# microsoft/fadtk

Hardware: NVIDIA H100
Metric: audio_seconds_embedded_per_second (higher is better)
Workload: dtype f16

## Files before the change

fadtk_b200/csrc/conv_gemm.cuh:

```cuda
#pragma once
#include "sm90.cuh"

namespace fad {

struct ConvGemmParams {
    int taps;
    int cblks;
    int box_w, box_h, box_n;
    int tiles_w, tiles_h;
    int img_groups;
    int n_tiles;
    int H, W, NB, Cout;
    float lo_scale;
    int lo8_group;
    int ld_out, n_valid;
    int relu, pool;
    const float* bias;
    __half* out;
    float* out_f32;
    uint8_t* out8;
    float* resid;
    int resid_C, resid_res, resid_shift;
};

// ... 1 lines not shown
    const int lg_nw = 28 - __clz(res);
    const int nw = res >> 3;
    const int in = (int)(o & 63);
    const long long wi = o >> 6;
    const int wx = (int)wi & (nw - 1);
    const int wy = (int)(wi >> lg_nw) & (nw - 1);
    const long long b = wi >> (2 * lg_nw);
    int y = wy * 8 + (in >> 3) + shift, xx = wx * 8 + (in & 7) + shift;
    if (y >= res) y -= res;
    if (xx >= res) xx -= res;
    return (b * res + y) * res + xx;
}

constexpr int kTileM = 128;
constexpr int kBlockK = 64;
constexpr int kConvGemmThreads = 384;
constexpr int kConsumers = 2;
constexpr int kChunkSteps = 8;
constexpr float kAccumShrinkPerElement = 1.06e-9f;
constexpr uint32_t kABytes = kTileM * kBlockK * 2;
constexpr uint32_t kEpiRowBytes = 128 * 4;
constexpr uint32_t kEpiBytes = 64 * kEpiRowBytes;
constexpr uint32_t kStagingBytes = 32 * 128;

template <int N_TILE, int WMODE>
__host__ __device__ constexpr uint32_t conv_gemm_stage_bytes() {
    return WMODE == 2 ? kABytes + N_TILE * kBlockK * 2 + N_TILE * kBlockK + kTileM * kBlockK
                      : kABytes + (WMODE == 1 ? 2 : 1) * N_TILE * kBlockK * 2;
}

template <int N_TILE, int STAGES, int WMODE>
__host__ __device__ constexpr uint32_t conv_gemm_smem_bytes() {
    return STAGES * conv_gemm_stage_bytes<N_TILE, WMODE>() + 1024  + 256
         + kConsumers * kEpiBytes;
}

__device__ __forceinline__ uint32_t pack_half2(float a, float b) {
    __half2 h = __floats2half2_rn(a, b);
    return *reinterpret_cast<uint32_t*>(&h);
}
__device__ __forceinline__ float gelu_erf(float x) {
    const float z = fminf(fabsf(x) * 0.70710678118654752f, 4.3f);
    float q = 1.04899843e-04f;
    q = fmaf(q, z, -4.92790774e-04f);
    q = fmaf(q, z, -2.22368206e-03f);
    q = fmaf(q, z, 2.93586859e-02f);
    q = fmaf(q, z, -1.48908889e-01f);
    q = fmaf(q, z, -9.18342944e-01f);
    q = fmaf(q, z, -1.62791250e+00f);
// ... 13 lines not shown
    __half2_raw h0, h1;
    h0.x = (unsigned short)(a & 0xffffu); h0.y = (unsigned short)(a >> 16);
    h1.x = (unsigned short)(b & 0xffffu); h1.y = (unsigned short)(b >> 16);
    return (uint32_t)__nv_cvt_halfraw2_to_fp8x2(h0, __NV_SATFINITE, __NV_E4M3)
         | ((uint32_t)__nv_cvt_halfraw2_to_fp8x2(h1, __NV_SATFINITE, __NV_E4M3) << 16);
}
__device__ __forceinline__ uint2 f16x8_to_e4m3x8(uint4 v) {
    return make_uint2(f16x4_to_e4m3x4(v.x, v.y), f16x4_to_e4m3x4(v.z, v.w));
}

__device__ __forceinline__ uint32_t hmax2_u32(uint32_t a, uint32_t b) {
    __half2 r = __hmax2(*reinterpret_cast<__half2*>(&a), *reinterpret_cast<__half2*>(&b));
    return *reinterpret_cast<uint32_t*>(&r);
}

template <int N_TILE, int STAGES, int WMODE>
__global__ void __launch_bounds__(kConvGemmThreads, 1)
conv_gemm_kernel(const __grid_constant__ CUtensorMap map_x,
                 const __grid_constant__ CUtensorMap map_w,
                 const __grid_constant__ CUtensorMap map_wl8,
                 const __grid_constant__ CUtensorMap map_x8,
                 const ConvGemmParams p)
{
    using namespace sm90;
    static_assert(N_TILE == 128, "one m64n128 accumulator per consumer warpgroup");
    constexpr bool SPLIT_W = WMODE == 1;
    constexpr bool LO8 = WMODE == 2;
    constexpr uint32_t kStageBytes = conv_gemm_stage_bytes<N_TILE, WMODE>();
    constexpr int kBRows = (WMODE != 0 ? 2 : 1) * N_TILE;
    constexpr uint32_t kWhBytes = N_TILE * kBlockK * 2;
    constexpr uint32_t kOffWl8 = kABytes + kWhBytes;
    constexpr uint32_t kOffA8 = kOffWl8 + N_TILE * kBlockK;
    constexpr int kColsPerThread = N_TILE / 2;
    constexpr int kGroups = kColsPerThread / 32;

    extern __shared__ uint8_t smem_raw[];
    uint8_t* smem = reinterpret_cast<uint8_t*>((reinterpret_cast<uintptr_t>(smem_raw) + 1023) & ~uintptr_t(1023));
    uint64_t* bars = reinterpret_cast<uint64_t*>(smem + STAGES * kStageBytes);
    uint64_t* full = bars;
    uint64_t* empty = bars + STAGES;
    uint8_t* epi = smem + STAGES * kStageBytes + 256;

    const int warp = threadIdx.x >> 5;
    const int lane = threadIdx.x & 31;
    const int ksteps = p.taps * p.cblks;
    const int n_chunks = (ksteps + kChunkSteps - 1) / kChunkSteps;
    const int chunk_len = (ksteps + n_chunks - 1) / n_chunks;
    const int m_tiles = p.img_groups * p.tiles_h * p.tiles_w;
    const int total_tiles = m_tiles * p.n_tiles;

    if (warp == 0 && lane == 0) {
        tma_prefetch_desc(&map_x);
        tma_prefetch_desc(&map_w);
        if (LO8) { tma_prefetch_desc(&map_wl8); tma_prefetch_desc(&map_x8); }
    }
    if (warp == 1 && lane == 0) {
        for (int s = 0; s < STAGES; ++s) { mbar_init(&full[s], 1); mbar_init(&empty[s], kConsumers * 4); }
        mbar_fence_init();
    }
    __syncthreads();

    if (warp < 4) {
        setmaxnreg_dec<40>();
        if (warp == 0 && elect_one()) {
            int s = 0; uint32_t ph = 0;
            for (int tile = blockIdx.x; tile < total_tiles; tile += gridDim.x) {
                const int nt = tile % p.n_tiles;
                const int m = tile / p.n_tiles;
                const int w0 = (m % p.tiles_w) * p.box_w;
                const int h0 = ((m / p.tiles_w) % p.tiles_h) * p.box_h;
                const int n0 = (m / (p.tiles_w * p.tiles_h)) * p.box_n;
                for (int ks = 0; ks < ksteps; ++ks) {
                    const int tap = ks / p.cblks;
                    const int cb = ks - tap * p.cblks;
                    int dh = 0, dw = 0;
                    if (p.taps == 9) { dh = tap / 3 - 1; dw = tap % 3 - 1; }
                    mbar_wait(&empty[s], ph ^ 1);
                    uint8_t* st = smem + s * kStageBytes;
                    mbar_expect_tx(&full[s], kStageBytes);
                    tma_load_4d(st, &map_x, &full[s], cb * kBlockK, w0 + dw, h0 + dh, n0);
                    tma_load_2d(st + kABytes, &map_w, &full[s], ks * kBlockK, nt * kBRows);
                    if (LO8) {
                        tma_load_2d(st + kOffWl8, &map_wl8, &full[s], ks * kBlockK, nt * N_TILE);
                        tma_load_4d(st + kOffA8, &map_x8, &full[s], cb * kBlockK, w0 + dw, h0 + dh, n0);
                    }
                    if (++s == STAGES) { s = 0; ph ^= 1; }
                }
            }
        }
    } else {
        setmaxnreg_inc<232>();
        const int c = (warp >> 2) - 1;
        const int wg_t = threadIdx.x & 127;
        const int wq = wg_t >> 5;
        const int rr = wg_t & 63;
        const int half = wg_t >> 6;
        const int r = c * 64 + rr;
        const int bw = p.box_w, bh = p.box_h;
        const int pw = r % bw;
        const int phh = (r / bw) % bh;
        const int pn = r / (bw * bh);
        const uint32_t epi_base = smem_u32(epi) + c * kEpiBytes;
        const uint32_t bar_id = 1 + c;
        int s = 0; uint32_t ph = 0;
        const bool plain = p.tiles_w == 1 && p.tiles_h == 1 && bw == 1 && bh == 1;
        auto prefetch_resid = [&](int nt_, int m_) {
            if (p.resid == nullptr || !plain) return;
            const int n_ = m_ * kTileM + r;
            if (n_ >= p.NB) return;
            const long long tok = p.resid_res ? window_row_to_token((long long)n_, p.resid_res, p.resid_shift) : (long long)n_;
            const int c0 = nt_ * N_TILE + half * kColsPerThread;
            for (int cc = c0; cc < c0 + kColsPerThread && cc < p.resid_C; cc += 32)
                asm volatile("prefetch.global.L2 [%0];" :: "l"(p.resid + tok * p.resid_C + cc));
        };
        if ((int)blockIdx.x < total_tiles) prefetch_resid((int)blockIdx.x % p.n_tiles, (int)blockIdx.x / p.n_tiles);
        auto load_bias = [&](float4 (&b)[8], int col0) {
            const float4* src = reinterpret_cast<const float4*>(p.bias + col0);
#pragma unroll
            for (int j = 0; j < 8; ++j) b[j] = __ldg(src + j);
        };

        for (int tile = blockIdx.x; tile < total_tiles; tile += gridDim.x) {
            const int nt = tile % p.n_tiles;
            const int m = tile / p.n_tiles;
            if (tile + (int)gridDim.x < total_tiles)
                prefetch_resid((tile + (int)gridDim.x) % p.n_tiles, (tile + (int)gridDim.x) / p.n_tiles);

            float sum[64], acc[64], corr[LO8 ? 64 : 1];
#pragma unroll
            for (int i = 0; i < 64; ++i) sum[i] = 0.f;
            for (int ks0 = 0; ks0 < ksteps; ks0 += chunk_len) {
                const int ks1 = min(ks0 + chunk_len, ksteps);
                const float unshrink = kAccumShrinkPerElement * (float)((ks1 - ks0) * kBlockK);
                int prev_s = -1;
                for (int ks = ks0; ks < ks1; ++ks) {
                    mbar_wait(&full[s], ph);
                    const uint32_t a_addr = smem_u32(smem + s * kStageBytes);
                    const uint64_t a_desc = kmajor_sw128_desc(a_addr + c * 64 * 128);
                    const uint64_t b_desc = kmajor_sw128_desc(a_addr + kABytes);
                    wgmma_fence();
#pragma unroll
                    for (int k = 0; k < kBlockK / 16; ++k) {
                        wgmma_m64n128k16_f16<0, 0>(acc, a_desc + 2 * k, b_desc + 2 * k, (ks > ks0) || (k > 0));
                        if (SPLIT_W)
                            wgmma_m64n128k16_f16<0, 0>(acc, a_desc + 2 * k, b_desc + 2 * k + (N_TILE * 128 / 16), 1);
                    }
                    if constexpr (LO8) {
                        const uint64_t a8_desc = kmajor_sw64_desc(a_addr + kOffA8 + c * 64 * 64);
                        const uint64_t w8_desc = kmajor_sw64_desc(a_addr + kOffWl8);
#pragma unroll
                        for (int k = 0; k < kBlockK / 32; ++k)
                            wgmma_m64n128k32_e4m3(corr, a8_desc + 2 * k, w8_desc + 2 * k, (ks > 0) || (k > 0));
                    }
                    wgmma_commit();
                    wgmma_wait<1>();
                    if (prev_s >= 0) { __syncwarp(); if (lane == 0) mbar_arrive(&empty[prev_s]); }
                    prev_s = s;
                    if (++s == STAGES) { s = 0; ph ^= 1; }
                }
                wgmma_wait<0>();
                fence_regs(acc);
                if constexpr (LO8) fence_regs(corr);
                __syncwarp();
                if (lane == 0) mbar_arrive(&empty[prev_s]);
#pragma unroll
                for (int i = 0; i < 64; ++i) sum[i] += fmaf(acc[i], unshrink, acc[i]);
            }
            if constexpr (LO8) {
#pragma unroll
                for (int i = 0; i < 64; ++i) sum[i] = fmaf(corr[i], p.lo_scale, sum[i]);
            }

            named_bar_sync(bar_id, 128);
            {
                const int fr = wq * 16 + (lane >> 2);
#pragma unroll
                for (int j = 0; j < 16; ++j) {
#pragma unroll
                    for (int i = 0; i < 2; ++i) {
                        const int row = fr + 8 * i, col = 8 * j + 2 * (lane & 3);
                        const uint32_t addr = epi_base + row * kEpiRowBytes + ((((col >> 2) ^ (row & 7))) << 4) + (col & 3) * 4;
                        sts64(addr, sum[4 * j + 2 * i], sum[4 * j + 2 * i + 1]);
                    }
                }
            }
            named_bar_sync(bar_id, 128);
            float accr[kColsPerThread];
#pragma unroll
            for (int q4 = 0; q4 < kColsPerThread / 4; ++q4) {
                const int ch = half * (kColsPerThread / 4) + q4;
                const uint4 u = lds128(epi_base + rr * kEpiRowBytes + ((ch ^ (rr & 7)) << 4));
                accr[4 * q4 + 0] = __uint_as_float(u.x); accr[4 * q4 + 1] = __uint_as_float(u.y);
                accr[4 * q4 + 2] = __uint_as_float(u.z); accr[4 * q4 + 3] = __uint_as_float(u.w);
            }
            named_bar_sync(bar_id, 128);

            int w, h, n;
            if (plain) { w = 0; h = 0; n = m * kTileM + r; }
            else {
                w = (m % p.tiles_w) * bw + pw;
                h = ((m / p.tiles_w) % p.tiles_h) * bh + phh;
                n = (m / (p.tiles_w * p.tiles_h)) * p.box_n + pn;
            }
            const bool valid = n < p.NB;
            const int ch0 = nt * N_TILE + half * kColsPerThread;
            long long out_off = -1, res_off = -1;
            if (valid && !p.pool) {
                out_off = (long long)((size_t(n) * p.H + h) * p.W + w) * p.ld_out;
                if (p.resid != nullptr)
                    res_off = (p.resid_res ? window_row_to_token((long long)n, p.resid_res, p.resid_shift) : (long long)n)
                              * p.resid_C;
            }
            const uint32_t stg = epi_base + wq * kStagingBytes;
            const uint32_t stg_mine = stg + lane * 128;
            const int sw = lane & 7;
            const int cq = lane & 7, rq = lane >> 3;
            const bool f32_path = p.out_f32 != nullptr || p.resid != nullptr;
            float4 bnext[8];
#pragma unroll
            for (int g = 0; g < kGroups; ++g) {
                float f[32];
                load_bias(bnext, ch0 + g * 32);
#pragma unroll
                for (int j = 0; j < 8; ++j) {
                    const float4 b = bnext[j];
                    f[4 * j + 0] = accr[g * 32 + 4 * j + 0] + b.x;
                    f[4 * j + 1] = accr[g * 32 + 4 * j + 1] + b.y;
                    f[4 * j + 2] = accr[g * 32 + 4 * j + 2] + b.z;
                    f[4 * j + 3] = accr[g * 32 + 4 * j + 3] + b.w;
                }
                if (p.relu == 1) {
#pragma unroll
                    for (int j = 0; j < 32; ++j) f[j] = fmaxf(f[j], 0.0f);
                } else if (p.relu == 2) {
#pragma unroll
                    for (int j = 0; j < 32; ++j) f[j] = gelu_erf(f[j]);
                } else if (p.relu == 3) {
#pragma unroll
                    for (int j = 0; j < 32; ++j) f[j] = elu_ex2(f[j]);
                }
                uint32_t h2[16];
#pragma unroll
                for (int j = 0; j < 16; ++j) h2[j] = pack_half2(f[2 * j], f[2 * j + 1]);

                if (!p.pool) {
                    if (f32_path) {
#pragma unroll
                        for (int j = 0; j < 8; ++j)
                            sts128(stg_mine + ((j ^ sw) << 4), __float_as_uint(f[4 * j]), __float_as_uint(f[4 * j + 1]),
                                   __float_as_uint(f[4 * j + 2]), __float_as_uint(f[4 * j + 3]));
                        __syncwarp();
                        float4 v[8];
#pragma unroll
                        for (int it = 0; it < 8; ++it) {
                            const int rr = it * 4 + rq;
                            const uint4 u = lds128(stg + rr * 128 + ((cq ^ (rr & 7)) << 4));
                            v[it] = make_float4(__uint_as_float(u.x), __uint_as_float(u.y), __uint_as_float(u.z), __uint_as_float(u.w));
                        }
                        const int col = ch0 + g * 32 + cq * 4;
                        if (p.out_f32 != nullptr) {
#pragma unroll
                            for (int it = 0; it < 8; ++it) {
                                const long long off = __shfl_sync(0xffffffffu, out_off, it * 4 + rq);
                                if (off >= 0 && col < p.n_valid) *reinterpret_cast<float4*>(p.out_f32 + off + col) = v[it];
                            }
                        }
                        if (p.resid != nullptr && ch0 + g * 32 < p.resid_C) {
#pragma unroll
                            for (int hf = 0; hf < 2; ++hf) {
                                long long offs[4];
                                float4 xv[4];
#pragma unroll
                                for (int it = 0; it < 4; ++it) {
                                    offs[it] = __shfl_sync(0xffffffffu, res_off, (hf * 4 + it) * 4 + rq);
                                    if (offs[it] >= 0) xv[it] = *reinterpret_cast<const float4*>(p.resid + offs[it] + col);
                                }
#pragma unroll
                                for (int it = 0; it < 4; ++it) {
                                    if (offs[it] >= 0) {
                                        const float4 a = v[hf * 4 + it];
                                        xv[it].x += a.x; xv[it].y += a.y; xv[it].z += a.z; xv[it].w += a.w;
                                        *reinterpret_cast<float4*>(p.resid + offs[it] + col) = xv[it];
                                    }
                                }
                            }
                        }
                        __syncwarp();
                        if (p.out != nullptr && out_off >= 0 && ch0 + g * 32 + 32 <= p.n_valid) {
                            uint4* dst = reinterpret_cast<uint4*>(p.out + out_off + ch0 + g * 32);
#pragma unroll
                            for (int j = 0; j < 4; ++j)
                                dst[j] = make_uint4(h2[4 * j], h2[4 * j + 1], h2[4 * j + 2], h2[4 * j + 3]);
                        }
                    } else if (p.out != nullptr) {
#pragma unroll
                        for (int j = 0; j < 4; ++j)
                            sts128(stg_mine + ((((g & 1) * 4 + j) ^ sw) << 4), h2[4 * j], h2[4 * j + 1], h2[4 * j + 2], h2[4 * j + 3]);
                        if (g & 1) {
                            __syncwarp();
                            const int col = ch0 + (g - 1) * 32 + cq * 8;
#pragma unroll
                            for (int it = 0; it < 8; ++it) {
                                const int rr = it * 4 + rq;
                                const uint4 v = lds128(stg + rr * 128 + ((cq ^ (rr & 7)) << 4));
                                const long long off = __shfl_sync(0xffffffffu, out_off, rr);
                                if (off >= 0 && col < p.n_valid) {
                                    *reinterpret_cast<uint4*>(p.out + off + col) = v;
                                    if (p.out8 != nullptr) *reinterpret_cast<uint2*>(p.out8 + off + col) = f16x8_to_e4m3x8(v);
                                }
                            }
                            __syncwarp();
                        }
                    }
                } else {
#pragma unroll
                    for (int j = 0; j < 16; ++j) {
                        uint32_t o = __shfl_xor_sync(0xffffffffu, h2[j], 1);
                        h2[j] = hmax2_u32(h2[j], o);
                        o = __shfl_xor_sync(0xffffffffu, h2[j], bw);
                        h2[j] = hmax2_u32(h2[j], o);
                    }
                    const int sub = (pw & 1) | ((phh & 1) << 1);
                    uint4 o;
                    o.x = sub == 0 ? h2[0] : sub == 1 ? h2[4] : sub == 2 ? h2[8]  : h2[12];
                    o.y = sub == 0 ? h2[1] : sub == 1 ? h2[5] : sub == 2 ? h2[9]  : h2[13];
                    o.z = sub == 0 ? h2[2] : sub == 1 ? h2[6] : sub == 2 ? h2[10] : h2[14];
                    o.w = sub == 0 ? h2[3] : sub == 1 ? h2[7] : sub == 2 ? h2[11] : h2[15];
                    if (valid) {
                        const size_t pix = (size_t(n) * (p.H >> 1) + (h >> 1)) * (p.W >> 1) + (w >> 1);
                        *reinterpret_cast<uint4*>(p.out + pix * p.Cout + ch0 + g * 32 + sub * 8) = o;
                        if (p.out8 != nullptr) *reinterpret_cast<uint2*>(p.out8 + pix * p.Cout + ch0 + g * 32 + sub * 8) = f16x8_to_e4m3x8(o);
                    }
                }
            }
        }
    }
}

}
```

fadtk_b200/csrc/fadtk_b200.cu:

```cuda
#include "../../include/fadtk_b200.h"

#include <cuda.h>
#include <cuda_runtime.h>
#include <cuda_fp16.h>
#include <cuda_fp8.h>
#include <algorithm>
#include <cmath>
#include <cstdio>
#include <cstdlib>
#include <cstring>
#include <map>
#include <string>
#include <vector>

#include "conv_gemm.cuh"
#include "frontend.cuh"
#include "stats.cuh"
#include "frechet.cuh"
#include "frechet_batched.cuh"
#include "clap.cuh"
#include "resample.cuh"
#include "whisper.cuh"
#include "encodec.cuh"
#include "wav2vec.cuh"
// ... 138 lines not shown
};

namespace {

template <int N_TILE, int STAGES, int WMODE>
int launch_conv_gemm(fad_handle* h, const CUtensorMap& mx, const CUtensorMap& mw, const CUtensorMap& mw8,
                     const CUtensorMap& mx8, const fad::ConvGemmParams& p, cudaStream_t st) {
    static bool attr_set = false;
    constexpr uint32_t smem = fad::conv_gemm_smem_bytes<N_TILE, STAGES, WMODE>();
    static_assert(smem <= 227 * 1024, "over the per-CTA shared-memory limit");
    auto kern = fad::conv_gemm_kernel<N_TILE, STAGES, WMODE>;
    if (!attr_set) {
        CK(cudaFuncSetAttribute(kern, cudaFuncAttributeMaxDynamicSharedMemorySize, (int)smem));
        attr_set = true;
    }
    const int total = p.img_groups * p.tiles_h * p.tiles_w * p.n_tiles;
    if (total == 0) return 0;
    const int grid = total < h->num_sms ? total : h->num_sms;
    kern<<<grid, fad::kConvGemmThreads, smem, st>>>(mx, mw, mw8, mx8, p);
    CK(cudaGetLastError());
    h->launches++;
    return 0;
}

int encode_layer_maps(const LayerGeom& g, const void* x, long long nb_dim, const void* w,
                      CUtensorMap* mx, CUtensorMap* mw, int a_cols = 0, long long a_row_stride = 0) {
    const uint64_t ac = a_cols > 0 ? (uint64_t)a_cols : (uint64_t)g.Cin;
    const uint64_t xd[4] = {ac, (uint64_t)g.W, (uint64_t)g.H, (uint64_t)nb_dim};
    uint64_t xs[3] = {ac * 2, (uint64_t)g.W * ac * 2, (uint64_t)g.H * g.W * ac * 2};
    if (a_row_stride > 0) xs[0] = xs[1] = xs[2] = (uint64_t)a_row_stride * 2;
    const uint32_t xb[4] = {64, (uint32_t)g.box_w, (uint32_t)g.box_h, (uint32_t)g.box_n};
    if (encode_f16_map(mx, x, 4, xd, xs, xb)) return 1;
    const uint64_t K = (uint64_t)g.taps * g.Cin;
    const uint64_t rows_mul = g.split_w ? 2 : 1;
    const uint64_t wd[2] = {K, (uint64_t)g.Cout * rows_mul};
    const uint64_t ws[1] = {K * 2};
    const uint32_t wb[2] = {64, (uint32_t)(g.n_tile * (g.split_w == 1 ? 2 : 1))};
    return encode_f16_map(mw, w, 2, wd, ws, wb);
}

int lo8_for(fad_handle* h, const LayerGeom& g, const void* w, CUtensorMap* mw8, float* inv_scale, cudaStream_t st);

bool attention_wgmma_enabled() {
    static const bool on = [] { const char* e = getenv("FADTK_ATTN"); return !(e && std::string(e) == "legacy"); }();
    return on;
}
int launch_attention_wgmma(fad_handle* h, const __half* qkv, long long n_clips, int S, int d, int heads, __half* out, cudaStream_t st) {
    static bool attr_set = false;
    if (!attr_set) {
        CK(cudaFuncSetAttribute(fad::attention_wgmma_kernel, cudaFuncAttributeMaxDynamicSharedMemorySize, (int)fad::kAtSmem));
        attr_set = true;
    }
// ... 977 lines not shown
```

fadtk_b200/csrc/sm90.cuh:

```cuda
#pragma once
#include <cuda.h>
#include <cuda_fp16.h>
#include <stdint.h>
#include <stdio.h>

namespace sm90 {

__device__ __forceinline__ uint32_t smem_u32(const void* p) {
    return static_cast<uint32_t>(__cvta_generic_to_shared(p));
}
__device__ __forceinline__ uint32_t lane_id() { return threadIdx.x & 31; }

__device__ __forceinline__ bool elect_one() {
    uint32_t pred;
    asm volatile(
        "{\n\t.reg .pred P;\n\t"
        "elect.sync _|P, 0xffffffff;\n\t"
        "selp.u32 %0, 1, 0, P;\n\t}\n"
        : "=r"(pred));
    return pred != 0;
}

template <uint32_t kRegs> __device__ __forceinline__ void setmaxnreg_inc() {
    asm volatile("setmaxnreg.inc.sync.aligned.u32 %0;" ::"n"(kRegs));
// ... 45 lines not shown
    asm volatile(
        "{\n\t.reg .pred P;\n\t"
        "mbarrier.try_wait.parity.shared::cta.b64 P, [%1], %2, %3;\n\t"
        "selp.u32 %0, 1, 0, P;\n\t}\n"
        : "=r"(ok) : "r"(smem_u32(bar)), "r"(parity), "r"(ns) : "memory");
    return ok != 0;
}
__device__ __forceinline__ void mbar_wait(uint64_t* bar, uint32_t parity) {
    if (mbar_try_wait(bar, parity)) return;
    uint32_t spins = 0;
    while (!mbar_try_wait_hint(bar, parity, 2000u)) {
        if (++spins > (1u << 24)) asm volatile("trap;");
    }
}

__device__ __forceinline__ void fence_proxy_async_smem() {
    asm volatile("fence.proxy.async.shared::cta;" ::: "memory");
}

__device__ __forceinline__ void tma_prefetch_desc(const CUtensorMap* m) {
    asm volatile("prefetch.tensormap [%0];" ::"l"(reinterpret_cast<uint64_t>(m)) : "memory");
}
__device__ __forceinline__ void tma_load_2d(void* dst, const CUtensorMap* m, uint64_t* bar,
                                            int c0, int c1) {
    asm volatile(
        "cp.async.bulk.tensor.2d.shared::cluster.global.mbarrier::complete_tx::bytes"
        " [%0], [%1, {%3, %4}], [%2];"
        ::"r"(smem_u32(dst)), "l"(reinterpret_cast<uint64_t>(m)), "r"(smem_u32(bar)),
          "r"(c0), "r"(c1) : "memory");
}
__device__ __forceinline__ void tma_load_3d(void* dst, const CUtensorMap* m, uint64_t* bar,
                                            int c0, int c1, int c2) {
    asm volatile(
        "cp.async.bulk.tensor.3d.shared::cluster.global.mbarrier::complete_tx::bytes"
        " [%0], [%1, {%3, %4, %5}], [%2];"
        ::"r"(smem_u32(dst)), "l"(reinterpret_cast<uint64_t>(m)), "r"(smem_u32(bar)),
          "r"(c0), "r"(c1), "r"(c2) : "memory");
}
__device__ __forceinline__ void tma_load_4d(void* dst, const CUtensorMap* m, uint64_t* bar,
                                            int c0, int c1, int c2, int c3) {
    asm volatile(
        "cp.async.bulk.tensor.4d.shared::cluster.global.mbarrier::complete_tx::bytes"
        " [%0], [%1, {%3, %4, %5, %6}], [%2];"
        ::"r"(smem_u32(dst)), "l"(reinterpret_cast<uint64_t>(m)), "r"(smem_u32(bar)),
// ... 84 lines not shown
```

Baseline: 127,200.

## Split conv GEMM into 2-CTA clusters with multicast weights and a dedicated epilogue warpgroup

For the f16 conv GEMM paths, the kernel now launches as 2-CTA clusters. Each CTA TMA-multicasts half of the weight tile to both CTAs, which roughly halves per-CTA weight traffic, and empty barriers are released across the cluster. A fourth warpgroup handles the epilogue (bias, activation, residual, stores) from a shared-memory tile handoff, so consumers can start the next tile's mainloop while the previous epilogue runs. Registers are rebalanced across producer, consumer and epilogue warps, and the epilogue prefetches residual rows into L2. The cost is cluster-level synchronisation, lower consumer register budgets, extra shared memory, and pairing M tiles, which can leave one CTA with padded work.

```diff
diff --git a/fadtk_b200/csrc/conv_gemm.cuh b/fadtk_b200/csrc/conv_gemm.cuh
--- a/fadtk_b200/csrc/conv_gemm.cuh
+++ b/fadtk_b200/csrc/conv_gemm.cuh
@@ -39,7 +39,6 @@
 
 constexpr int kTileM = 128;
 constexpr int kBlockK = 64;
-constexpr int kConvGemmThreads = 384;
 constexpr int kConsumers = 2;
 constexpr int kChunkSteps = 8;
 constexpr float kAccumShrinkPerElement = 1.06e-9f;
@@ -47,6 +46,11 @@
 constexpr uint32_t kEpiRowBytes = 128 * 4;
 constexpr uint32_t kEpiBytes = 64 * kEpiRowBytes;
 constexpr uint32_t kStagingBytes = 32 * 128;
+constexpr uint32_t kRegsProducer = 24, kRegsConsumer = 184, kRegsEpilogue = 120;
+static_assert(128 * (kRegsProducer + 2 * kRegsConsumer + kRegsEpilogue) <= 65536, "register split over the register file");
+
+template <int WMODE>
+__host__ __device__ constexpr int conv_gemm_threads() { return WMODE == 2 ? 384 : 512; }
 
 template <int N_TILE, int WMODE>
 __host__ __device__ constexpr uint32_t conv_gemm_stage_bytes() {
@@ -57,7 +61,7 @@
 template <int N_TILE, int STAGES, int WMODE>
 __host__ __device__ constexpr uint32_t conv_gemm_smem_bytes() {
     return STAGES * conv_gemm_stage_bytes<N_TILE, WMODE>() + 1024  + 256
-         + kConsumers * kEpiBytes;
+         + kConsumers * kEpiBytes + (WMODE == 2 ? 0 : 4 * kStagingBytes);
 }
 
 __device__ __forceinline__ uint32_t pack_half2(float a, float b) {
@@ -101,20 +105,342 @@
     return *reinterpret_cast<uint32_t*>(&r);
 }
 
-template <int N_TILE, int STAGES, int WMODE>
-__global__ void __launch_bounds__(kConvGemmThreads, 1)
-conv_gemm_kernel(const __grid_constant__ CUtensorMap map_x,
-                 const __grid_constant__ CUtensorMap map_w,
-                 const __grid_constant__ CUtensorMap map_wl8,
-                 const __grid_constant__ CUtensorMap map_x8,
-                 const ConvGemmParams p)
+struct EpiRow {
+    long long out_off, res_off;
+    int n, h, w, pw, phh;
+    bool valid;
+};
+
+template <int N_TILE>
+__device__ __forceinline__ EpiRow epilogue_row(const ConvGemmParams& p, bool plain, int m, int r) {
+    EpiRow e;
+    const int bw = p.box_w, bh = p.box_h;
+    e.pw = r % bw;
+    e.phh = (r / bw) % bh;
+    if (plain) { e.w = 0; e.h = 0; e.n = m * kTileM + r; }
+    else {
+        e.w = (m % p.tiles_w) * bw + e.pw;
+        e.h = ((m / p.tiles_w) % p.tiles_h) * bh + e.phh;
+        e.n = (m / (p.tiles_w * p.tiles_h)) * p.box_n + r / (bw * bh);
+    }
+    e.valid = e.n < p.NB;
+    e.out_off = -1; e.res_off = -1;
+    if (e.valid && !p.pool) {
+        e.out_off = (long long)((size_t(e.n) * p.H + e.h) * p.W + e.w) * p.ld_out;
+        if (p.resid != nullptr)
+            e.res_off = (p.resid_res ? window_row_to_token((long long)e.n, p.resid_res, p.resid_shift) : (long long)e.n)
+                        * p.resid_C;
+    }
+    return e;
+}
+
+__device__ __forceinline__ void prefetch_resid(const ConvGemmParams& p, bool plain, int m, int r, int c0, int cols) {
+    if (p.resid == nullptr || !plain) return;
+    const int n = m * kTileM + r;
+    if (n >= p.NB) return;
+    const long long tok = p.resid_res ? window_row_to_token((long long)n, p.resid_res, p.resid_shift) : (long long)n;
+    for (int cc = c0; cc < c0 + cols && cc < p.resid_C; cc += 32)
+        asm volatile("prefetch.global.L2 [%0];" :: "l"(p.resid + tok * p.resid_C + cc));
+}
+
+__device__ __forceinline__ void epilogue_group(const ConvGemmParams& p, const float (&a)[32], int col, bool odd,
+                                               const EpiRow& e, uint32_t stg, int lane) {
+    using namespace sm90;
+    const uint32_t stg_mine = stg + lane * 128;
+    const int sw = lane & 7;
+    const int cq = lane & 7, rq = lane >> 3;
+    const bool f32_path = p.out_f32 != nullptr || p.resid != nullptr;
+    float f[32];
+    float4 bnext[8];
+    {
+        const float4* src = reinterpret_cast<const float4*>(p.bias + col);
+#pragma unroll
+        for (int j = 0; j < 8; ++j) bnext[j] = __ldg(src + j);
+    }
+#pragma unroll
+    for (int j = 0; j < 8; ++j) {
+        const float4 b = bnext[j];
+        f[4 * j + 0] = a[4 * j + 0] + b.x;
+        f[4 * j + 1] = a[4 * j + 1] + b.y;
+        f[4 * j + 2] = a[4 * j + 2] + b.z;
+        f[4 * j + 3] = a[4 * j + 3] + b.w;
+    }
+    if (p.relu == 1) {
+#pragma unroll
+        for (int j = 0; j < 32; ++j) f[j] = fmaxf(f[j], 0.0f);
+    } else if (p.relu == 2) {
+#pragma unroll
+        for (int j = 0; j < 32; ++j) f[j] = gelu_erf(f[j]);
+    } else if (p.relu == 3) {
+#pragma unroll
+        for (int j = 0; j < 32; ++j) f[j] = elu_ex2(f[j]);
+    }
+    uint32_t h2[16];
+#pragma unroll
+    for (int j = 0; j < 16; ++j) h2[j] = pack_half2(f[2 * j], f[2 * j + 1]);
+
+    if (!p.pool) {
+        if (f32_path) {
+#pragma unroll
+            for (int j = 0; j < 8; ++j)
+                sts128(stg_mine + ((j ^ sw) << 4), __float_as_uint(f[4 * j]), __float_as_uint(f[4 * j + 1]),
+                       __float_as_uint(f[4 * j + 2]), __float_as_uint(f[4 * j + 3]));
+            __syncwarp();
+            float4 v[8];
+#pragma unroll
+            for (int it = 0; it < 8; ++it) {
+                const int rr = it * 4 + rq;
+                const uint4 u = lds128(stg + rr * 128 + ((cq ^ (rr & 7)) << 4));
+                v[it] = make_float4(__uint_as_float(u.x), __uint_as_float(u.y), __uint_as_float(u.z), __uint_as_float(u.w));
+            }
+            const int c = col + cq * 4;
+            if (p.out_f32 != nullptr) {
+#pragma unroll
+                for (int it = 0; it < 8; ++it) {
+                    const long long off = __shfl_sync(0xffffffffu, e.out_off, it * 4 + rq);
+                    if (off >= 0 && c < p.n_valid) *reinterpret_cast<float4*>(p.out_f32 + off + c) = v[it];
+                }
+            }
+            if (p.resid != nullptr && col < p.resid_C) {
+#pragma unroll
+                for (int hf = 0; hf < 2; ++hf) {
+                    long long offs[4];
+                    float4 xv[4];
+#pragma unroll
+                    for (int it = 0; it < 4; ++it) {
+                        offs[it] = __shfl_sync(0xffffffffu, e.res_off, (hf * 4 + it) * 4 + rq);
+                        if (offs[it] >= 0) xv[it] = *reinterpret_cast<const float4*>(p.resid + offs[it] + c);
+                    }
+#pragma unroll
+                    for (int it = 0; it < 4; ++it) {
+                        if (offs[it] >= 0) {
+                            const float4 av = v[hf * 4 + it];
+                            xv[it].x += av.x; xv[it].y += av.y; xv[it].z += av.z; xv[it].w += av.w;
+                            *reinterpret_cast<float4*>(p.resid + offs[it] + c) = xv[it];
+                        }
+                    }
+                }
+            }
+            __syncwarp();
+            if (p.out != nullptr && e.out_off >= 0 && col + 32 <= p.n_valid) {
+                uint4* dst = reinterpret_cast<uint4*>(p.out + e.out_off + col);
+#pragma unroll
+                for (int j = 0; j < 4; ++j)
+                    dst[j] = make_uint4(h2[4 * j], h2[4 * j + 1], h2[4 * j + 2], h2[4 * j + 3]);
+            }
+        } else if (p.out != nullptr) {
+#pragma unroll
+            for (int j = 0; j < 4; ++j)
+                sts128(stg_mine + ((((odd ? 4 : 0) + j) ^ sw) << 4), h2[4 * j], h2[4 * j + 1], h2[4 * j + 2], h2[4 * j + 3]);
+            if (odd) {
+                __syncwarp();
+                const int c = col - 32 + cq * 8;
+#pragma unroll
+                for (int it = 0; it < 8; ++it) {
+                    const int rr = it * 4 + rq;
+                    const uint4 v = lds128(stg + rr * 128 + ((cq ^ (rr & 7)) << 4));
+                    const long long off = __shfl_sync(0xffffffffu, e.out_off, rr);
+                    if (off >= 0 && c < p.n_valid) {
+                        *reinterpret_cast<uint4*>(p.out + off + c) = v;
+                        if (p.out8 != nullptr) *reinterpret_cast<uint2*>(p.out8 + off + c) = f16x8_to_e4m3x8(v);
+                    }
+                }
+                __syncwarp();
+            }
+        }
+    } else {
+#pragma unroll
+        for (int j = 0; j < 16; ++j) {
+            uint32_t o = __shfl_xor_sync(0xffffffffu, h2[j], 1);
+            h2[j] = hmax2_u32(h2[j], o);
+            o = __shfl_xor_sync(0xffffffffu, h2[j], p.box_w);
+            h2[j] = hmax2_u32(h2[j], o);
+        }
+        const int sub = (e.pw & 1) | ((e.phh & 1) << 1);
+        uint4 o;
+        o.x = sub == 0 ? h2[0] : sub == 1 ? h2[4] : sub == 2 ? h2[8]  : h2[12];
+        o.y = sub == 0 ? h2[1] : sub == 1 ? h2[5] : sub == 2 ? h2[9]  : h2[13];
+        o.z = sub == 0 ? h2[2] : sub == 1 ? h2[6] : sub == 2 ? h2[10] : h2[14];
+        o.w = sub == 0 ? h2[3] : sub == 1 ? h2[7] : sub == 2 ? h2[11] : h2[15];
+        if (e.valid) {
+            const size_t pix = (size_t(e.n) * (p.H >> 1) + (e.h >> 1)) * (p.W >> 1) + (e.w >> 1);
+            *reinterpret_cast<uint4*>(p.out + pix * p.Cout + col + sub * 8) = o;
+            if (p.out8 != nullptr) *reinterpret_cast<uint2*>(p.out8 + pix * p.Cout + col + sub * 8) = f16x8_to_e4m3x8(o);
+        }
+    }
+}
+
+__device__ __forceinline__ void store_fragment(uint32_t base, const float (&sum)[64], int wq, int lane) {
+    using namespace sm90;
+    const int fr = wq * 16 + (lane >> 2);
+#pragma unroll
+    for (int j = 0; j < 16; ++j) {
+#pragma unroll
+        for (int i = 0; i < 2; ++i) {
+            const int row = fr + 8 * i, col = 8 * j + 2 * (lane & 3);
+            const uint32_t addr = base + row * kEpiRowBytes + ((((col >> 2) ^ (row & 7))) << 4) + (col & 3) * 4;
+            sts64(addr, sum[4 * j + 2 * i], sum[4 * j + 2 * i + 1]);
+        }
+    }
+}
+
+__device__ __forceinline__ void load_row32(float (&a)[32], uint32_t base, int row, int ch0) {
+    using namespace sm90;
+#pragma unroll
+    for (int q4 = 0; q4 < 8; ++q4) {
+        const uint4 u = lds128(base + row * kEpiRowBytes + (((ch0 + q4) ^ (row & 7)) << 4));
+        a[4 * q4 + 0] = __uint_as_float(u.x); a[4 * q4 + 1] = __uint_as_float(u.y);
+        a[4 * q4 + 2] = __uint_as_float(u.z); a[4 * q4 + 3] = __uint_as_float(u.w);
+    }
+}
+
+template <int N_TILE, int STAGES, bool SPLIT_W>
+__device__ __forceinline__ void conv_gemm_f16(const CUtensorMap& map_x, const CUtensorMap& map_w, const ConvGemmParams& p)
 {
     using namespace sm90;
-    static_assert(N_TILE == 128, "one m64n128 accumulator per consumer warpgroup");
-    constexpr bool SPLIT_W = WMODE == 1;
-    constexpr bool LO8 = WMODE == 2;
-    constexpr uint32_t kStageBytes = conv_gemm_stage_bytes<N_TILE, WMODE>();
-    constexpr int kBRows = (WMODE != 0 ? 2 : 1) * N_TILE;
+    constexpr uint32_t kStageBytes = conv_gemm_stage_bytes<N_TILE, SPLIT_W ? 1 : 0>();
+    constexpr int kBRows = (SPLIT_W ? 2 : 1) * N_TILE;
+
+    extern __shared__ uint8_t smem_raw[];
+    uint8_t* smem = reinterpret_cast<uint8_t*>((reinterpret_cast<uintptr_t>(smem_raw) + 1023) & ~uintptr_t(1023));
+    uint64_t* bars = reinterpret_cast<uint64_t*>(smem + STAGES * kStageBytes);
+    uint64_t* full = bars;
+    uint64_t* empty = bars + STAGES;
+    uint64_t* tile_full = bars + 2 * STAGES;
+    uint64_t* tile_free = tile_full + 1;
+    constexpr uint32_t kWHalfBytes = kBRows / 2 * kBlockK * 2;
+    const uint32_t epi = smem_u32(smem + STAGES * kStageBytes + 256);
+    const uint32_t staging = epi + kConsumers * kEpiBytes;
+
+    const int warp = threadIdx.x >> 5;
+    const int lane = threadIdx.x & 31;
+    const int ksteps = p.taps * p.cblks;
+    const int n_chunks = (ksteps + kChunkSteps - 1) / kChunkSteps;
+    const int chunk_len = (ksteps + n_chunks - 1) / n_chunks;
+    const int m_tiles = p.img_groups * p.tiles_h * p.tiles_w;
+    const int n_pairs = (m_tiles + 1) / 2 * p.n_tiles;
+    const uint32_t rank = cluster_ctarank();
+    const int first_pair = (int)cluster_id_x(), pair_stride = (int)cluster_count_x();
+
+    if (warp == 0 && lane == 0) {
+        tma_prefetch_desc(&map_x);
+        tma_prefetch_desc(&map_w);
+    }
+    if (warp == 1 && lane == 0) {
+        for (int s = 0; s < STAGES; ++s) { mbar_init(&full[s], 1); mbar_init(&empty[s], 2 * kConsumers * 4); }
+        mbar_init(tile_full, kConsumers * 128);
+        mbar_init(tile_free, 128);
+        mbar_fence_init();
+    }
+    cluster_sync();
+
+    if (warp < 4) {
+        setmaxnreg_dec<kRegsProducer>();
+        if (warp == 0 && elect_one()) {
+            int s = 0; uint32_t ph = 0;
+            for (int q = first_pair; q < n_pairs; q += pair_stride) {
+                const int nt = q % p.n_tiles;
+                const int m = 2 * (q / p.n_tiles) + (int)rank;
+                const int w0 = (m % p.tiles_w) * p.box_w;
+                const int h0 = ((m / p.tiles_w) % p.tiles_h) * p.box_h;
+                const int n0 = (m / (p.tiles_w * p.tiles_h)) * p.box_n;
+                for (int ks = 0; ks < ksteps; ++ks) {
+                    const int tap = ks / p.cblks;
+                    const int cb = ks - tap * p.cblks;
+                    int dh = 0, dw = 0;
+                    if (p.taps == 9) { dh = tap / 3 - 1; dw = tap % 3 - 1; }
+                    mbar_wait(&empty[s], ph ^ 1);
+                    uint8_t* st = smem + s * kStageBytes;
+                    mbar_expect_tx(&full[s], kStageBytes);
+                    tma_load_4d(st, &map_x, &full[s], cb * kBlockK, w0 + dw, h0 + dh, n0);
+                    tma_load_2d_multicast(st + kABytes + rank * kWHalfBytes, &map_w, &full[s], ks * kBlockK,
+                                          nt * kBRows + (int)rank * (kBRows / 2), 0x3);
+                    if (++s == STAGES) { s = 0; ph ^= 1; }
+                }
+            }
+        }
+    } else if (warp < 12) {
+        setmaxnreg_inc<kRegsConsumer>();
+        const int c = (warp >> 2) - 1;
+        const int wq = warp & 3;
+        int s = 0; uint32_t ph = 0, tph = 0;
+        for (int q = first_pair; q < n_pairs; q += pair_stride) {
+            float sum[64], acc[64];
+#pragma unroll
+            for (int i = 0; i < 64; ++i) sum[i] = 0.f;
+            for (int ks0 = 0; ks0 < ksteps; ks0 += chunk_len) {
+                const int ks1 = min(ks0 + chunk_len, ksteps);
+                const float unshrink = kAccumShrinkPerElement * (float)((ks1 - ks0) * kBlockK);
+                int prev_s = -1;
+                for (int ks = ks0; ks < ks1; ++ks) {
+                    mbar_wait(&full[s], ph);
+                    const uint32_t a_addr = smem_u32(smem + s * kStageBytes);
+                    const uint64_t a_desc = kmajor_sw128_desc(a_addr + c * 64 * 128);
+                    const uint64_t b_desc = kmajor_sw128_desc(a_addr + kABytes);
+                    wgmma_fence();
+#pragma unroll
+                    for (int k = 0; k < kBlockK / 16; ++k) {
+                        wgmma_m64n128k16_f16<0, 0>(acc, a_desc + 2 * k, b_desc + 2 * k, (ks > ks0) || (k > 0));
+                        if (SPLIT_W)
+                            wgmma_m64n128k16_f16<0, 0>(acc, a_desc + 2 * k, b_desc + 2 * k + (N_TILE * 128 / 16), 1);
+                    }
+                    wgmma_commit();
+                    wgmma_wait<1>();
+                    if (prev_s >= 0) {
+                        __syncwarp();
+                        if (lane == 0) { mbar_arrive(&empty[prev_s]); mbar_arrive_cluster(&empty[prev_s], rank ^ 1); }
+                    }
+                    prev_s = s;
+                    if (++s == STAGES) { s = 0; ph ^= 1; }
+                }
+                wgmma_wait<0>();
+                fence_regs(acc);
+                __syncwarp();
+                if (lane == 0) { mbar_arrive(&empty[prev_s]); mbar_arrive_cluster(&empty[prev_s], rank ^ 1); }
+#pragma unroll
+                for (int i = 0; i < 64; ++i) sum[i] += fmaf(acc[i], unshrink, acc[i]);
+            }
+            mbar_wait(tile_free, tph ^ 1);
+            store_fragment(epi + c * kEpiBytes, sum, wq, lane);
+            mbar_arrive(tile_full);
+            tph ^= 1;
+        }
+    } else {
+        setmaxnreg_dec<kRegsEpilogue>();
+        const int r = threadIdx.x & 127;
+        const uint32_t half_base = epi + (r >> 6) * kEpiBytes;
+        const int hr = r & 63;
+        const uint32_t stg = staging + (warp & 3) * kStagingBytes;
+        const bool plain = p.tiles_w == 1 && p.tiles_h == 1 && p.box_w == 1 && p.box_h == 1;
+        uint32_t tph = 0;
+        if (first_pair < n_pairs)
+            prefetch_resid(p, plain, 2 * (first_pair / p.n_tiles) + (int)rank, r, (first_pair % p.n_tiles) * N_TILE, N_TILE);
+        for (int q = first_pair; q < n_pairs; q += pair_stride) {
+            const int nt = q % p.n_tiles;
+            const int m = 2 * (q / p.n_tiles) + (int)rank;
+            const int next = q + pair_stride;
+            if (next < n_pairs) prefetch_resid(p, plain, 2 * (next / p.n_tiles) + (int)rank, r, (next % p.n_tiles) * N_TILE, N_TILE);
+            const EpiRow e = epilogue_row<N_TILE>(p, plain, m, r);
+            mbar_wait(tile_full, tph);
+            tph ^= 1;
+#pragma unroll 1
+            for (int g = 0; g < N_TILE / 32; ++g) {
+                float a[32];
+                load_row32(a, half_base, hr, g * 8);
+                if (g == N_TILE / 32 - 1) mbar_arrive(tile_free);
+                epilogue_group(p, a, nt * N_TILE + g * 32, g & 1, e, stg, lane);
+            }
+        }
+    }
+    cluster_sync();
+}
+
+template <int N_TILE, int STAGES>
+__device__ __forceinline__ void conv_gemm_lo8(const CUtensorMap& map_x, const CUtensorMap& map_w,
+                                              const CUtensorMap& map_wl8, const CUtensorMap& map_x8, const ConvGemmParams& p)
+{
+    using namespace sm90;
+    constexpr uint32_t kStageBytes = conv_gemm_stage_bytes<N_TILE, 2>();
     constexpr uint32_t kWhBytes = N_TILE * kBlockK * 2;
     constexpr uint32_t kOffWl8 = kABytes + kWhBytes;
     constexpr uint32_t kOffA8 = kOffWl8 + N_TILE * kBlockK;
@@ -139,7 +465,8 @@
     if (warp == 0 && lane == 0) {
         tma_prefetch_desc(&map_x);
         tma_prefetch_desc(&map_w);
-        if (LO8) { tma_prefetch_desc(&map_wl8); tma_prefetch_desc(&map_x8); }
+        tma_prefetch_desc(&map_wl8);
+        tma_prefetch_desc(&map_x8);
     }
     if (warp == 1 && lane == 0) {
         for (int s = 0; s < STAGES; ++s) { mbar_init(&full[s], 1); mbar_init(&empty[s], kConsumers * 4); }
@@ -166,11 +493,9 @@
                     uint8_t* st = smem + s * kStageBytes;
                     mbar_expect_tx(&full[s], kStageBytes);
                     tma_load_4d(st, &map_x, &full[s], cb * kBlockK, w0 + dw, h0 + dh, n0);
-                    tma_load_2d(st + kABytes, &map_w, &full[s], ks * kBlockK, nt * kBRows);
-                    if (LO8) {
-                        tma_load_2d(st + kOffWl8, &map_wl8, &full[s], ks * kBlockK, nt * N_TILE);
-                        tma_load_4d(st + kOffA8, &map_x8, &full[s], cb * kBlockK, w0 + dw, h0 + dh, n0);
-                    }
+                    tma_load_2d(st + kABytes, &map_w, &full[s], ks * kBlockK, nt * N_TILE * 2);
+                    tma_load_2d(st + kOffWl8, &map_wl8, &full[s], ks * kBlockK, nt * N_TILE);
+                    tma_load_4d(st + kOffA8, &map_x8, &full[s], cb * kBlockK, w0 + dw, h0 + dh, n0);
                     if (++s == STAGES) { s = 0; ph ^= 1; }
                 }
             }
@@ -183,37 +508,22 @@
         const int rr = wg_t & 63;
         const int half = wg_t >> 6;
         const int r = c * 64 + rr;
-        const int bw = p.box_w, bh = p.box_h;
-        const int pw = r % bw;
-        const int phh = (r / bw) % bh;
-        const int pn = r / (bw * bh);
         const uint32_t epi_base = smem_u32(epi) + c * kEpiBytes;
         const uint32_t bar_id = 1 + c;
         int s = 0; uint32_t ph = 0;
-        const bool plain = p.tiles_w == 1 && p.tiles_h == 1 && bw == 1 && bh == 1;
-        auto prefetch_resid = [&](int nt_, int m_) {
-            if (p.resid == nullptr || !plain) return;
-            const int n_ = m_ * kTileM + r;
-            if (n_ >= p.NB) return;
-            const long long tok = p.resid_res ? window_row_to_token((long long)n_, p.resid_res, p.resid_shift) : (long long)n_;
-            const int c0 = nt_ * N_TILE + half * kColsPerThread;
-            for (int cc = c0; cc < c0 + kColsPerThread && cc < p.resid_C; cc += 32)
-                asm volatile("prefetch.global.L2 [%0];" :: "l"(p.resid + tok * p.resid_C + cc));
-        };
-        if ((int)blockIdx.x < total_tiles) prefetch_resid((int)blockIdx.x % p.n_tiles, (int)blockIdx.x / p.n_tiles);
-        auto load_bias = [&](float4 (&b)[8], int col0) {
-            const float4* src = reinterpret_cast<const float4*>(p.bias + col0);
-#pragma unroll
-            for (int j = 0; j < 8; ++j) b[j] = __ldg(src + j);
-        };
+        const bool plain = p.tiles_w == 1 && p.tiles_h == 1 && p.box_w == 1 && p.box_h == 1;
+        if ((int)blockIdx.x < total_tiles)
+            prefetch_resid(p, plain, (int)blockIdx.x / p.n_tiles, r, ((int)blockIdx.x % p.n_tiles) * N_TILE + half * kColsPerThread,
+                           kColsPerThread);
 
         for (int tile = blockIdx.x; tile < total_tiles; tile += gridDim.x) {
             const int nt = tile % p.n_tiles;
             const int m = tile / p.n_tiles;
-            if (tile + (int)gridDim.x < total_tiles)
-                prefetch_resid((tile + (int)gridDim.x) % p.n_tiles, (tile + (int)gridDim.x) / p.n_tiles);
-
-            float sum[64], acc[64], corr[LO8 ? 64 : 1];
+            const int next = tile + (int)gridDim.x;
+            if (next < total_tiles)
+                prefetch_resid(p, plain, next / p.n_tiles, r, (next % p.n_tiles) * N_TILE + half * kColsPerThread, kColsPerThread);
+
+            float sum[64], acc[64], corr[64];
 #pragma unroll
             for (int i = 0; i < 64; ++i) sum[i] = 0.f;
             for (int ks0 = 0; ks0 < ksteps; ks0 += chunk_len) {
@@ -227,18 +537,13 @@
                     const uint64_t b_desc = kmajor_sw128_desc(a_addr + kABytes);
                     wgmma_fence();
 #pragma unroll
-                    for (int k = 0; k < kBlockK / 16; ++k) {
+                    for (int k = 0; k < kBlockK / 16; ++k)
                         wgmma_m64n128k16_f16<0, 0>(acc, a_desc + 2 * k, b_desc + 2 * k, (ks > ks0) || (k > 0));
-                        if (SPLIT_W)
-                            wgmma_m64n128k16_f16<0, 0>(acc, a_desc + 2 * k, b_desc + 2 * k + (N_TILE * 128 / 16), 1);
-                    }
-                    if constexpr (LO8) {
-                        const uint64_t a8_desc = kmajor_sw64_desc(a_addr + kOffA8 + c * 64 * 64);
-                        const uint64_t w8_desc = kmajor_sw64_desc(a_addr + kOffWl8);
-#pragma unroll
-                        for (int k = 0; k < kBlockK / 32; ++k)
-                            wgmma_m64n128k32_e4m3(corr, a8_desc + 2 * k, w8_desc + 2 * k, (ks > 0) || (k > 0));
-                    }
+                    const uint64_t a8_desc = kmajor_sw64_desc(a_addr + kOffA8 + c * 64 * 64);
+                    const uint64_t w8_desc = kmajor_sw64_desc(a_addr + kOffWl8);
+#pragma unroll
+                    for (int k = 0; k < kBlockK / 32; ++k)
+                        wgmma_m64n128k32_e4m3(corr, a8_desc + 2 * k, w8_desc + 2 * k, (ks > 0) || (k > 0));
                     wgmma_commit();
                     wgmma_wait<1>();
                     if (prev_s >= 0) { __syncwarp(); if (lane == 0) mbar_arrive(&empty[prev_s]); }
@@ -247,181 +552,52 @@
                 }
                 wgmma_wait<0>();
                 fence_regs(acc);
-                if constexpr (LO8) fence_regs(corr);
+                fence_regs(corr);
                 __syncwarp();
                 if (lane == 0) mbar_arrive(&empty[prev_s]);
 #pragma unroll
                 for (int i = 0; i < 64; ++i) sum[i] += fmaf(acc[i], unshrink, acc[i]);
             }
-            if constexpr (LO8) {
-#pragma unroll
-                for (int i = 0; i < 64; ++i) sum[i] = fmaf(corr[i], p.lo_scale, sum[i]);
-            }
+#pragma unroll
+            for (int i = 0; i < 64; ++i) sum[i] = fmaf(corr[i], p.lo_scale, sum[i]);
 
             named_bar_sync(bar_id, 128);
-            {
-                const int fr = wq * 16 + (lane >> 2);
-#pragma unroll
-                for (int j = 0; j < 16; ++j) {
-#pragma unroll
-                    for (int i = 0; i < 2; ++i) {
-                        const int row = fr + 8 * i, col = 8 * j + 2 * (lane & 3);
-                        const uint32_t addr = epi_base + row * kEpiRowBytes + ((((col >> 2) ^ (row & 7))) << 4) + (col & 3) * 4;
-                        sts64(addr, sum[4 * j + 2 * i], sum[4 * j + 2 * i + 1]);
-                    }
-                }
-            }
+            store_fragment(epi_base, sum, wq, lane);
             named_bar_sync(bar_id, 128);
             float accr[kColsPerThread];
 #pragma unroll
-            for (int q4 = 0; q4 < kColsPerThread / 4; ++q4) {
-                const int ch = half * (kColsPerThread / 4) + q4;
-                const uint4 u = lds128(epi_base + rr * kEpiRowBytes + ((ch ^ (rr & 7)) << 4));
-                accr[4 * q4 + 0] = __uint_as_float(u.x); accr[4 * q4 + 1] = __uint_as_float(u.y);
-                accr[4 * q4 + 2] = __uint_as_float(u.z); accr[4 * q4 + 3] = __uint_as_float(u.w);
+            for (int g = 0; g < kGroups; ++g) {
+                float a[32];
+                load_row32(a, epi_base, rr, half * (kColsPerThread / 4) + g * 8);
+#pragma unroll
+                for (int i = 0; i < 32; ++i) accr[g * 32 + i] = a[i];
             }
             named_bar_sync(bar_id, 128);
 
-            int w, h, n;
-            if (plain) { w = 0; h = 0; n = m * kTileM + r; }
-            else {
-                w = (m % p.tiles_w) * bw + pw;
-                h = ((m / p.tiles_w) % p.tiles_h) * bh + phh;
-                n = (m / (p.tiles_w * p.tiles_h)) * p.box_n + pn;
-            }
-            const bool valid = n < p.NB;
-            const int ch0 = nt * N_TILE + half * kColsPerThread;
-            long long out_off = -1, res_off = -1;
-            if (valid && !p.pool) {
-                out_off = (long long)((size_t(n) * p.H + h) * p.W + w) * p.ld_out;
-                if (p.resid != nullptr)
-                    res_off = (p.resid_res ? window_row_to_token((long long)n, p.resid_res, p.resid_shift) : (long long)n)
-                              * p.resid_C;
-            }
+            const EpiRow e = epilogue_row<N_TILE>(p, plain, m, r);
             const uint32_t stg = epi_base + wq * kStagingBytes;
-            const uint32_t stg_mine = stg + lane * 128;
-            const int sw = lane & 7;
-            const int cq = lane & 7, rq = lane >> 3;
-            const bool f32_path = p.out_f32 != nullptr || p.resid != nullptr;
-            float4 bnext[8];
 #pragma unroll
             for (int g = 0; g < kGroups; ++g) {
-                float f[32];
-                load_bias(bnext, ch0 + g * 32);
-#pragma unroll
-                for (int j = 0; j < 8; ++j) {
-                    const float4 b = bnext[j];
-                    f[4 * j + 0] = accr[g * 32 + 4 * j + 0] + b.x;
-                    f[4 * j + 1] = accr[g * 32 + 4 * j + 1] + b.y;
-                    f[4 * j + 2] = accr[g * 32 + 4 * j + 2] + b.z;
-                    f[4 * j + 3] = accr[g * 32 + 4 * j + 3] + b.w;
-                }
-                if (p.relu == 1) {
-#pragma unroll
-                    for (int j = 0; j < 32; ++j) f[j] = fmaxf(f[j], 0.0f);
-                } else if (p.relu == 2) {
-#pragma unroll
-                    for (int j = 0; j < 32; ++j) f[j] = gelu_erf(f[j]);
-                } else if (p.relu == 3) {
-#pragma unroll
-                    for (int j = 0; j < 32; ++j) f[j] = elu_ex2(f[j]);
-                }
-                uint32_t h2[16];
-#pragma unroll
-                for (int j = 0; j < 16; ++j) h2[j] = pack_half2(f[2 * j], f[2 * j + 1]);
-
-                if (!p.pool) {
-                    if (f32_path) {
-#pragma unroll
-                        for (int j = 0; j < 8; ++j)
-                            sts128(stg_mine + ((j ^ sw) << 4), __float_as_uint(f[4 * j]), __float_as_uint(f[4 * j + 1]),
-                                   __float_as_uint(f[4 * j + 2]), __float_as_uint(f[4 * j + 3]));
-                        __syncwarp();
-                        float4 v[8];
-#pragma unroll
-                        for (int it = 0; it < 8; ++it) {
-                            const int rr = it * 4 + rq;
-                            const uint4 u = lds128(stg + rr * 128 + ((cq ^ (rr & 7)) << 4));
-                            v[it] = make_float4(__uint_as_float(u.x), __uint_as_float(u.y), __uint_as_float(u.z), __uint_as_float(u.w));
-                        }
-                        const int col = ch0 + g * 32 + cq * 4;
-                        if (p.out_f32 != nullptr) {
-#pragma unroll
-                            for (int it = 0; it < 8; ++it) {
-                                const long long off = __shfl_sync(0xffffffffu, out_off, it * 4 + rq);
-                                if (off >= 0 && col < p.n_valid) *reinterpret_cast<float4*>(p.out_f32 + off + col) = v[it];
-                            }
-                        }
-                        if (p.resid != nullptr && ch0 + g * 32 < p.resid_C) {
-#pragma unroll
-                            for (int hf = 0; hf < 2; ++hf) {
-                                long long offs[4];
-                                float4 xv[4];
-#pragma unroll
-                                for (int it = 0; it < 4; ++it) {
-                                    offs[it] = __shfl_sync(0xffffffffu, res_off, (hf * 4 + it) * 4 + rq);
-                                    if (offs[it] >= 0) xv[it] = *reinterpret_cast<const float4*>(p.resid + offs[it] + col);
-                                }
-#pragma unroll
-                                for (int it = 0; it < 4; ++it) {
-                                    if (offs[it] >= 0) {
-                                        const float4 a = v[hf * 4 + it];
-                                        xv[it].x += a.x; xv[it].y += a.y; xv[it].z += a.z; xv[it].w += a.w;
-                                        *reinterpret_cast<float4*>(p.resid + offs[it] + col) = xv[it];
-                                    }
-                                }
-                            }
-                        }
-                        __syncwarp();
-                        if (p.out != nullptr && out_off >= 0 && ch0 + g * 32 + 32 <= p.n_valid) {
-                            uint4* dst = reinterpret_cast<uint4*>(p.out + out_off + ch0 + g * 32);
-#pragma unroll
-                            for (int j = 0; j < 4; ++j)
-                                dst[j] = make_uint4(h2[4 * j], h2[4 * j + 1], h2[4 * j + 2], h2[4 * j + 3]);
-                        }
-                    } else if (p.out != nullptr) {
-#pragma unroll
-                        for (int j = 0; j < 4; ++j)
-                            sts128(stg_mine + ((((g & 1) * 4 + j) ^ sw) << 4), h2[4 * j], h2[4 * j + 1], h2[4 * j + 2], h2[4 * j + 3]);
-                        if (g & 1) {
-                            __syncwarp();
-                            const int col = ch0 + (g - 1) * 32 + cq * 8;
-#pragma unroll
-                            for (int it = 0; it < 8; ++it) {
-                                const int rr = it * 4 + rq;
-                                const uint4 v = lds128(stg + rr * 128 + ((cq ^ (rr & 7)) << 4));
-                                const long long off = __shfl_sync(0xffffffffu, out_off, rr);
-                                if (off >= 0 && col < p.n_valid) {
-                                    *reinterpret_cast<uint4*>(p.out + off + col) = v;
-                                    if (p.out8 != nullptr) *reinterpret_cast<uint2*>(p.out8 + off + col) = f16x8_to_e4m3x8(v);
-                                }
-                            }
-                            __syncwarp();
-                        }
-                    }
-                } else {
-#pragma unroll
-                    for (int j = 0; j < 16; ++j) {
-                        uint32_t o = __shfl_xor_sync(0xffffffffu, h2[j], 1);
-                        h2[j] = hmax2_u32(h2[j], o);
-                        o = __shfl_xor_sync(0xffffffffu, h2[j], bw);
-                        h2[j] = hmax2_u32(h2[j], o);
-                    }
-                    const int sub = (pw & 1) | ((phh & 1) << 1);
-                    uint4 o;
-                    o.x = sub == 0 ? h2[0] : sub == 1 ? h2[4] : sub == 2 ? h2[8]  : h2[12];
-                    o.y = sub == 0 ? h2[1] : sub == 1 ? h2[5] : sub == 2 ? h2[9]  : h2[13];
-                    o.z = sub == 0 ? h2[2] : sub == 1 ? h2[6] : sub == 2 ? h2[10] : h2[14];
-                    o.w = sub == 0 ? h2[3] : sub == 1 ? h2[7] : sub == 2 ? h2[11] : h2[15];
-                    if (valid) {
-                        const size_t pix = (size_t(n) * (p.H >> 1) + (h >> 1)) * (p.W >> 1) + (w >> 1);
-                        *reinterpret_cast<uint4*>(p.out + pix * p.Cout + ch0 + g * 32 + sub * 8) = o;
-                        if (p.out8 != nullptr) *reinterpret_cast<uint2*>(p.out8 + pix * p.Cout + ch0 + g * 32 + sub * 8) = f16x8_to_e4m3x8(o);
-                    }
-                }
-            }
-        }
-    }
-}
-
-}
+                float a[32];
+#pragma unroll
+                for (int i = 0; i < 32; ++i) a[i] = accr[g * 32 + i];
+                epilogue_group(p, a, nt * N_TILE + half * kColsPerThread + g * 32, g & 1, e, stg, lane);
+            }
+        }
+    }
+}
+
+template <int N_TILE, int STAGES, int WMODE>
+__global__ void __launch_bounds__(conv_gemm_threads<WMODE>(), 1)
+conv_gemm_kernel(const __grid_constant__ CUtensorMap map_x,
+                 const __grid_constant__ CUtensorMap map_w,
+                 const __grid_constant__ CUtensorMap map_wl8,
+                 const __grid_constant__ CUtensorMap map_x8,
+                 const ConvGemmParams p)
+{
+    static_assert(N_TILE == 128, "one m64n128 accumulator per consumer warpgroup");
+    if constexpr (WMODE == 2) conv_gemm_lo8<N_TILE, STAGES>(map_x, map_w, map_wl8, map_x8, p);
+    else conv_gemm_f16<N_TILE, STAGES, WMODE == 1>(map_x, map_w, p);
+}
+
+}
diff --git a/fadtk_b200/csrc/fadtk_b200.cu b/fadtk_b200/csrc/fadtk_b200.cu
--- a/fadtk_b200/csrc/fadtk_b200.cu
+++ b/fadtk_b200/csrc/fadtk_b200.cu
@@ -176,10 +176,32 @@
         CK(cudaFuncSetAttribute(kern, cudaFuncAttributeMaxDynamicSharedMemorySize, (int)smem));
         attr_set = true;
     }
-    const int total = p.img_groups * p.tiles_h * p.tiles_w * p.n_tiles;
-    if (total == 0) return 0;
-    const int grid = total < h->num_sms ? total : h->num_sms;
-    kern<<<grid, fad::kConvGemmThreads, smem, st>>>(mx, mw, mw8, mx8, p);
+    const int m_tiles = p.img_groups * p.tiles_h * p.tiles_w;
+    if (m_tiles * p.n_tiles == 0) return 0;
+    if constexpr (WMODE == 2) {
+        const int total = m_tiles * p.n_tiles;
+        const int grid = total < h->num_sms ? total : h->num_sms;
+        kern<<<grid, fad::conv_gemm_threads<WMODE>(), smem, st>>>(mx, mw, mw8, mx8, p);
+    } else {
+        cudaLaunchConfig_t cfg = {};
+        cudaLaunchAttribute attr[1];
+        attr[0].id = cudaLaunchAttributeClusterDimension;
+        attr[0].val.clusterDim.x = 2; attr[0].val.clusterDim.y = 1; attr[0].val.clusterDim.z = 1;
+        cfg.blockDim = dim3(fad::conv_gemm_threads<WMODE>());
+        cfg.dynamicSmemBytes = smem;
+        cfg.stream = st;
+        cfg.attrs = attr;
+        cfg.numAttrs = 1;
+        static int max_clusters = 0;
+        if (max_clusters == 0) {
+            cfg.gridDim = dim3(2 * h->num_sms);
+            CK(cudaOccupancyMaxActiveClusters(&max_clusters, kern, &cfg));
+            if (max_clusters <= 0) return fail("conv_gemm_kernel: no 2-CTA cluster fits on this device");
+        }
+        const int n_pairs = (m_tiles + 1) / 2 * p.n_tiles;
+        cfg.gridDim = dim3(2 * (n_pairs < max_clusters ? n_pairs : max_clusters));
+        CK(cudaLaunchKernelEx(&cfg, kern, mx, mw, mw8, mx8, p));
+    }
     CK(cudaGetLastError());
     h->launches++;
     return 0;
@@ -197,7 +219,7 @@
     const uint64_t rows_mul = g.split_w ? 2 : 1;
     const uint64_t wd[2] = {K, (uint64_t)g.Cout * rows_mul};
     const uint64_t ws[1] = {K * 2};
-    const uint32_t wb[2] = {64, (uint32_t)(g.n_tile * (g.split_w == 1 ? 2 : 1))};
+    const uint32_t wb[2] = {64, (uint32_t)(g.split_w == 2 ? g.n_tile : g.n_tile * (g.split_w == 1 ? 2 : 1) / 2)};
     return encode_f16_map(mw, w, 2, wd, ws, wb);
 }
 
diff --git a/fadtk_b200/csrc/sm90.cuh b/fadtk_b200/csrc/sm90.cuh
--- a/fadtk_b200/csrc/sm90.cuh
+++ b/fadtk_b200/csrc/sm90.cuh
@@ -83,6 +83,30 @@
     }
 }
 
+__device__ __forceinline__ uint32_t cluster_ctarank() {
+    uint32_t r;
+    asm volatile("mov.u32 %0, %%cluster_ctarank;" : "=r"(r));
+    return r;
+}
+__device__ __forceinline__ uint32_t cluster_id_x() {
+    uint32_t r;
+    asm volatile("mov.u32 %0, %%clusterid.x;" : "=r"(r));
+    return r;
+}
+__device__ __forceinline__ uint32_t cluster_count_x() {
+    uint32_t r;
+    asm volatile("mov.u32 %0, %%nclusterid.x;" : "=r"(r));
+    return r;
+}
+__device__ __forceinline__ void cluster_arrive() { asm volatile("barrier.cluster.arrive.release;" ::: "memory"); }
+__device__ __forceinline__ void cluster_wait() { asm volatile("barrier.cluster.wait.acquire;" ::: "memory"); }
+__device__ __forceinline__ void cluster_sync() { cluster_arrive(); cluster_wait(); }
+__device__ __forceinline__ void mbar_arrive_cluster(uint64_t* bar, uint32_t rank) {
+    uint32_t remote;
+    asm volatile("mapa.shared::cluster.u32 %0, %1, %2;" : "=r"(remote) : "r"(smem_u32(bar)), "r"(rank));
+    asm volatile("mbarrier.arrive.shared::cluster.b64 _, [%0];" ::"r"(remote) : "memory");
+}
+
 __device__ __forceinline__ void fence_proxy_async_smem() {
     asm volatile("fence.proxy.async.shared::cta;" ::: "memory");
 }
@@ -97,6 +121,14 @@
         " [%0], [%1, {%3, %4}], [%2];"
         ::"r"(smem_u32(dst)), "l"(reinterpret_cast<uint64_t>(m)), "r"(smem_u32(bar)),
           "r"(c0), "r"(c1) : "memory");
+}
+__device__ __forceinline__ void tma_load_2d_multicast(void* dst, const CUtensorMap* m, uint64_t* bar,
+                                                      int c0, int c1, uint16_t cta_mask) {
+    asm volatile(
+        "cp.async.bulk.tensor.2d.shared::cluster.global.mbarrier::complete_tx::bytes.multicast::cluster"
+        " [%0], [%1, {%3, %4}], [%2], %5;"
+        ::"r"(smem_u32(dst)), "l"(reinterpret_cast<uint64_t>(m)), "r"(smem_u32(bar)),
+          "r"(c0), "r"(c1), "h"(cta_mask) : "memory");
 }
 __device__ __forceinline__ void tma_load_3d(void* dst, const CUtensorMap* m, uint64_t* bar,
                                             int c0, int c1, int c2) {
```

Result: faster. 141,300 (median of 6 runs) (+11.1%).
